# CederGroupHub/chgnet

Measured on NVIDIA H100. Metric: structures_per_sec_EFS, higher is better.
Workload: dtype f32

## Files before the change

chgnet_b200/_lib.py:

```python
from __future__ import annotations

import ctypes
import os
from ctypes import c_char_p, c_float, c_int32, c_int64, c_void_p

import torch
from torch import Tensor

_HERE = os.path.dirname(os.path.abspath(__file__))
LIB_PATH = os.path.join(_HERE, "libchgnet_b200.so")

P, I, F, I64 = c_void_p, c_int32, c_float, c_int64

SIGNATURES: dict[str, list] = {
    "chg_embed_atoms": [P, P, I, P, P],
    "chg_edge_geometry": [P, P, P, P, P, P, I, P, P, P, P],
    "chg_bond_basis_embed": [P, P, I, P, P, I, F, F, I, P, P, P, P, P, P],
    "chg_bond_basis_bwd": [P, P, I, P, P, I, F, F, I, P, P, P, P, P, P, P],
    "chg_angle_basis_embed": [P, P, P, I, P, I, P, P, P, P],
    "chg_angle_basis_bwd": [P, P, P, I, P, I, P, P, P, P, P],
    "chg_linear": [P, P, I, I, P, P, P, P, I, P, P],
    "chg_gather_rows": [P, P, I, I, P, P],
    "chg_scatter_rows": [P, P, I, I, P, P],
    "chg_atom_conv_fwd": [P, P, P, P, P, P, I, P, P, P, P, P, P, P],
    "chg_atom_conv_bwd": [P, P, P, P, P, P, I, P, P, P, P, P, P, P, P, P],
    "chg_segment_sum": [P, I, P, P, I, I, I, P, I, P],
    "chg_atom_conv_fused": [P, P, P, P, P, P, P, I, I, P, P, P, P, P, P, P],
    "chg_bond_conv_fused": [P, P, P, P, P, P, P, P, I, I, P, P, P, P, P, P, P, P],
    "chg_bond_conv_fwd": [P, P, P, P, P, P, P, I, P, P, P, P, P, P, P],
    "chg_bond_conv_bwd": [P, P, P, P, P, I, P, P, P, P, P, P, P, P, P],
    "chg_angle_update_fwd": [P, P, P, P, P, P, P, I, P, P, P, P],
    "chg_angle_update_bwd": [P, P, I, P, P, P, P],
    "chg_readout": [P, P, P, I, P, P, P, P, I, P, F, P, P, P, P, P, P, P],
    "chg_magmom": [P, I, P, F, P, P],
    "chg_force_virial": [P, P, P, P, P, P, P, P, P, P, I, P, P, P],
    "chg_wgrad": [P, P, I, P, I, P, I, P, I, I, P, I, P, P, P],
    "chg_colsum": [P, I, P, I, P, I, I, P, P],
    "chg_readout_bwd": [P, I, P, P, P, P, I, P, P, P, P, P, P, P, P],
    "chg_magmom_bwd": [P, I, P, F, P, P, P, P],
    "chg_loss_terms": [P, P, I, I, F, P, P, P],
    "chg_adam_step": [P, P, P, P, I64, F, F, F, F, F, I, P],
    "chg_edge_tangent": [P, P, P, P, P, P, P, P, I, P, P, P],
    "chg_bond_basis_tangent": [P, P, P, I, P, P, I, F, F, I, P, P, P, P, P, P],
    "chg_bond_basis_bwd2": [P, P, P, I, P, P, I, F, F, I, P, P, P, P, P, P],
    "chg_angle_basis_tangent": [P, P, P, P, I, P, I, P, P, P, P],
    "chg_angle_basis_bwd2": [P, P, P, P, I, P, I, P, P, P, P],
    "chg_atom_conv_tan": [P, P, P, P, P, P, P, I, P, P, P, P, P, P, P, P],
# ... 169 lines not shown

    def segment_sum(self, data, perm, ptr, accumulate, out):
        self._chk(data, perm, ptr)
        if not out.is_cuda or out.stride(1) != 1:
            raise ChgnetB200Error("segment_sum output must be a CUDA tensor with unit column stride")
        n_items = data.shape[0] if perm is None else perm.shape[0]
        self._call("chg_segment_sum", _p(data), data.shape[1], _p(perm), _p(ptr), ptr.shape[0] - 1, n_items,
                   int(accumulate), _p(out), out.stride(0))

    def bond_conv_fwd(self, pij, px, pa, wbg, ang_atom, ang_i, ang_j, w2t, b2, ln, upd, save_pre, save_p):
        self._chk(pij, px, pa, wbg, ang_atom, ang_i, ang_j, w2t, b2, ln, upd, save_pre, save_p)
        self._call("chg_bond_conv_fwd", _p(pij), _p(px), _p(pa), _p(wbg), _p(ang_atom), _p(ang_i), _p(ang_j),
                   ang_i.shape[0], _p(w2t), _p(b2), _p(ln), _p(upd), _p(save_pre), _p(save_p))

    def bond_conv_bwd(self, save_pre, save_p, wbg, ang_i, ang_j, g_agg, w2, ln, g_pre, gw_i, gw_j, g_p=None,
                      g_ln=None):
        self._chk(save_pre, save_p, wbg, ang_i, ang_j, g_agg, w2, ln, g_pre, gw_i, gw_j, g_p, g_ln)
        self._call("chg_bond_conv_bwd", _p(save_pre), _p(save_p), _p(wbg), _p(ang_i), _p(ang_j), ang_i.shape[0],
                   _p(g_agg), _p(w2), _p(ln), _p(g_pre), _p(gw_i), _p(gw_j), _p(g_p), _p(g_ln))

    def angle_update_fwd(self, pij, px, pa, ang, ang_atom, ang_i, ang_j, ln, ang_new, save_p):
        self._chk(pij, px, pa, ang, ang_atom, ang_i, ang_j, ln, ang_new, save_p)
        self._call("chg_angle_update_fwd", _p(pij), _p(px), _p(pa), _p(ang), _p(ang_atom), _p(ang_i), _p(ang_j),
                   ang_i.shape[0], _p(ln), _p(ang_new), _p(save_p))

    def angle_update_bwd(self, save_p, g_ang_in, ln, g_pre, g_ln=None):
        self._chk(save_p, g_ang_in, ln, g_pre, g_ln)
        self._call("chg_angle_update_bwd", _p(save_p), _p(g_ang_in), save_p.shape[0], _p(ln), _p(g_pre), _p(g_ln))

    @staticmethod
    def _chk_rows(*tensors: Tensor | None) -> None:
        for t in tensors:
            if t is not None and (not t.is_cuda or t.stride(-1) != 1):
                raise ChgnetB200Error("kernel arguments must be CUDA tensors with unit column stride")

    def _workspace(self, n_out: int, device) -> Tensor:
        ws = getattr(self, "_ws", None)
        if ws is None or ws.device != device:
            need = max(int(self.lib.chg_wgrad_workspace_floats(n)) for n in (64, 128, 256))
            ws = torch.empty(need, dtype=torch.float32, device=device)
            self._ws = ws
# ... 151 lines not shown
```

chgnet_b200/csrc/gated.cu:

```cuda
#include <cstdlib>

#include "gated_common.cuh"

namespace chg {
namespace {

using namespace gated;

template <int MODE>
struct FwdSmem {
  static constexpr bool HAS_W2 = MODE != ANGLE;
  static constexpr int W2_OFF = 0;
  static constexpr int TILE_OFF = W2_OFF + (HAS_W2 ? 64 * 128 : 0);
  static constexpr int TILE_FLOATS = HAS_W2 ? TM * HS : 0;
  static constexpr int B2_OFF = TILE_OFF + TILE_FLOATS;
  static constexpr int LN_OFF = B2_OFF + 128;
  static constexpr int IDX_OFF = LN_OFF + 256;
  static constexpr int TOTAL_BYTES = (IDX_OFF + 3 * TM) * 4;
};

template <int MODE>
__global__ void __launch_bounds__(NTHR, 2) gated_fwd_kernel(const FwdArgs a) {
  using L = FwdSmem<MODE>;
  extern __shared__ __align__(16) float smem[];
// ... 125 lines not shown
  const int tid = threadIdx.x;
  const int tx = tid & 15, ty = tid >> 4;
  const int r0 = ty * 4, c0 = tx * 4;
  const bool use_ln = a.ln != nullptr;

  if (L::HAS_W2) copy_to_smem(s_w2, a.w2, 128 * 64, tid);
  if (use_ln) s_ln[tid] = a.ln[tid];
  float ln_acc[16];
#pragma unroll
  for (int j = 0; j < 16; ++j) ln_acc[j] = 0.f;

  const int n_tiles = (a.n_rows + TM - 1) / TM;
  for (int tile = blockIdx.x; tile < n_tiles; tile += gridDim.x) {
    const int base = tile * TM;
    __syncthreads();
    if (MODE != ANGLE && tid < TM) {
      const int r = min(base + tid, a.n_rows - 1);
      s_idx[tid] = a.idx0[r];
      s_idx[TM + tid] = a.idx1[r];
      if (MODE == ATOM) s_idx[2 * TM + tid] = a.idx2[r];
    }
    __syncthreads();

    float4 g1, g2, b1, b2v;
    if (use_ln) {
      g1 = lds4(s_ln + c0);
      b1 = lds4(s_ln + 64 + c0);
      g2 = lds4(s_ln + 128 + c0);
      b2v = lds4(s_ln + 192 + c0);
    }
#pragma unroll
    for (int i = 0; i < 4; ++i) {
      const int row = r0 + i;
      const int g = base + row;
      const bool valid = g < a.n_rows;
      const int r = min(g, a.n_rows - 1);
      const float4 pc4 = ldg4(a.save_p + (size_t)r * 128 + c0);
      const float4 pg4 = ldg4(a.save_p + (size_t)r * 128 + 64 + c0);
      float y1[4] = {pc4.x, pc4.y, pc4.z, pc4.w};
      float y2[4] = {pg4.x, pg4.y, pg4.z, pg4.w};
      float xh1[4], xh2[4], rstd1 = 1.f, rstd2 = 1.f;
      if (use_ln) {
        ln_stats(y1, xh1, rstd1);
        ln_stats(y2, xh2, rstd2);
#pragma unroll
        for (int j = 0; j < 4; ++j) {
          y1[j] = fmaf(xh1[j], f4at(g1, j), f4at(b1, j));
          y2[j] = fmaf(xh2[j], f4at(g2, j), f4at(b2v, j));
        }
      }
      float s1[4], core[4], gate[4];
      float4 o;
#pragma unroll
// ... 579 lines not shown
  CHG_CHECK_ARG(pij && px && pa && ang && ang_atom && ang_i && ang_j && ang_new, "null pointer");
  FwdArgs a{pij, px, pa, ang, nullptr, ang_i, ang_j, ang_atom, n_angles, nullptr, nullptr, ln, ang_new,
            nullptr, save_p};
  return launch_fwd<ANGLE>(a, as_stream(stream));
}

extern "C" int chg_angle_update_bwd(const float* save_p, const float* g_ang_in, int32_t n_angles, const float* ln,
                                    float* g_pre, double* g_ln, void* stream) {
  CHG_CHECK_ARG(n_angles >= 0, "negative size");
  if (n_angles == 0) return CHG_OK;
  CHG_CHECK_ARG(save_p && g_pre, "null pointer");
  BwdArgs a{nullptr, nullptr, nullptr, nullptr, nullptr, nullptr, n_angles, nullptr, save_p, g_ang_in,
            nullptr, ln, g_pre, nullptr, nullptr, nullptr, g_ln};
  return launch_bwd<ANGLE>(a, as_stream(stream));
}
```

chgnet_b200/csrc/gated_common.cuh:

```cuda
#pragma once
#include "common.cuh"

namespace chg {
namespace gated {

constexpr int HS = 132;
constexpr float LN_EPS = 1e-5f;
}
int ws_min_rows();
namespace gated {

enum Mode { ATOM = 0, BOND = 1, ANGLE = 2 };

struct FwdArgs {
  const float* p_a;
  const float* p_b;
  const float* p_c;
  const float* feat;
  const float* wgt;
  const int32_t* idx0;
  const int32_t* idx1;
  const int32_t* idx2;
  int32_t n_rows;
  const float* w2t;
// ... 10 lines not shown
  const float* wgt;
  const int32_t* idx0;
  const int32_t* idx1;
  const int32_t* idx2;
  int32_t n_rows;
  const float* save_pre;
  const float* save_p;
  const float* g_in;
  const float* w2;
  const float* ln;
  float* g_pre;
  float* g_w0;
  float* g_w1;
  float* g_p;
  double* g_ln;
};

__device__ __forceinline__ void ln_stats(const float (&v)[4], float (&xhat)[4], float& rstd) {
  const float mean = sum16(v[0] + v[1] + v[2] + v[3]) * (1.f / 64.f);
  float d[4], ss = 0.f;
#pragma unroll
  for (int j = 0; j < 4; ++j) {
    d[j] = v[j] - mean;
    ss = fmaf(d[j], d[j], ss);
  }
  const float var = sum16(ss) * (1.f / 64.f);
  rstd = 1.f / sqrtf(var + LN_EPS);
#pragma unroll
  for (int j = 0; j < 4; ++j) xhat[j] = d[j] * rstd;
}
// ... 94 lines not shown
```

chgnet_b200/csrc/gated_ws.cu:

```cuda
#include "gated_common.cuh"
#include "tc.cuh"

namespace chg {
namespace gated {
namespace {

constexpr int WS_THREADS = 512;
constexpr int TR = 128;
constexpr int HALF_BYTES = TR * 64 * 4;
constexpr int IMG_BYTES = 64 * 64 * 4;
constexpr int STRIP = 16;

struct WsSmem {
  static constexpr int IMG_OFF = 0;
  static constexpr int HS_OFF = 4 * IMG_BYTES;
  static constexpr int O_OFF = HS_OFF + 2 * HALF_BYTES;
  static constexpr int GIDX_OFF = O_OFF + HALF_BYTES;
  static constexpr int EIDX_OFF = GIDX_OFF + 2 * 3 * TR * 4;
  static constexpr int B2_OFF = EIDX_OFF + 4 * TR * 4;
  static constexpr int LN_OFF = B2_OFF + 128 * 4;
  static constexpr int TOTAL = LN_OFF + 256 * 4;
};

struct WsBars {
// ... 353 lines not shown
struct WsBwdSmem {
  static constexpr int IMG_OFF = 0;
  static constexpr int T1_OFF = 4 * IMG_BYTES;
  static constexpr int T2_OFF = T1_OFF + 2 * HALF_BYTES;
  static constexpr int PIDX_OFF = T2_OFF + 2 * HALF_BYTES;
  static constexpr int FIDX_OFF = PIDX_OFF + 3 * TR * 4;
  static constexpr int LN_OFF = FIDX_OFF + 3 * TR * 4;
  static constexpr int TOTAL = LN_OFF + 256 * 4;
};

struct WsBwdBars {
  uint64_t a_full, a_empty;
};

template <int MODE>
__global__ void __launch_bounds__(WS_THREADS, 1) gated_ws_bwd_kernel(const BwdArgs a) {
  extern __shared__ __align__(1024) uint8_t smem_raw[];
  uint8_t* s_img = smem_raw + WsBwdSmem::IMG_OFF;
  uint8_t* s_t1 = smem_raw + WsBwdSmem::T1_OFF;
  uint8_t* s_t2 = smem_raw + WsBwdSmem::T2_OFF;
  int* s_pidx = reinterpret_cast<int*>(smem_raw + WsBwdSmem::PIDX_OFF);
  int* s_fidx = reinterpret_cast<int*>(smem_raw + WsBwdSmem::FIDX_OFF);
  float* s_ln = reinterpret_cast<float*>(smem_raw + WsBwdSmem::LN_OFF);
  __shared__ __align__(8) WsBwdBars bars;

  const int tid = threadIdx.x, warp = tid >> 5;
  const bool use_ln = a.ln != nullptr;
  const int n_tiles = (a.n_rows + TR - 1) / TR;

  build_image_ws(s_img, s_img + IMG_BYTES, a.w2, 64, 0, tid);
// ... 34 lines not shown
      if (use_ln) {
        g1 = lds4(s_ln + c0);
        b1 = lds4(s_ln + 64 + c0);
        g2 = lds4(s_ln + 128 + c0);
        b2v = lds4(s_ln + 192 + c0);
      }
      tc::mbar_wait(&bars.a_empty, (tl & 1) ^ 1);
#pragma unroll 2
      for (int pass = 0; pass < 8; ++pass) {
        const int row = pass * 16 + ty;
        const int g = base + row;
        const bool valid = g < a.n_rows;
        const int r = min(g, a.n_rows - 1);
        const float4 pc4 = ldg4(a.save_p + (size_t)r * 128 + c0);
        const float4 pg4 = ldg4(a.save_p + (size_t)r * 128 + 64 + c0);
        float4 gm, wv;
        if (MODE == ATOM) {
          gm = ldg4(a.g_in + (size_t)s_pidx[row] * 64 + c0);
          wv = ldg4(a.wgt + (size_t)s_pidx[2 * TR + row] * 64 + c0);
        } else {
          gm = ldg4(a.g_in + (size_t)s_pidx[row] * 64 + c0);
          wv = ldg4(a.wgt + (size_t)s_pidx[row] * 64 + c0);
        }
        float y1[4] = {pc4.x, pc4.y, pc4.z, pc4.w};
        float y2[4] = {pg4.x, pg4.y, pg4.z, pg4.w};
        float xh1[4], xh2[4], rstd1 = 1.f, rstd2 = 1.f;
        if (use_ln) {
          ln_stats(y1, xh1, rstd1);
          ln_stats(y2, xh2, rstd2);
#pragma unroll
          for (int j = 0; j < 4; ++j) {
            y1[j] = fmaf(xh1[j], f4at(g1, j), f4at(b1, j));
            y2[j] = fmaf(xh2[j], f4at(g2, j), f4at(b2v, j));
          }
        }
        float s1[4], core[4], gate[4];
        float4 o;
#pragma unroll
        for (int j = 0; j < 4; ++j) {
          s1[j] = sigmoid_f(y1[j]);
          core[j] = y1[j] * s1[j];
          gate[j] = sigmoid_f(y2[j]);
          f4at(o, j) = core[j] * gate[j];
        }
        float4 go;
        if (MODE == ATOM) {
          if (valid) stg4(a.g_w0 + (size_t)g * 64 + c0, gm * o);
          go = gm * wv;
        } else {
          const float4 wj = ldg4(a.wgt + (size_t)s_pidx[TR + row] * 64 + c0);
          const float4 gmo = gm * o;
          if (valid) {
            stg4(a.g_w0 + (size_t)g * 64 + c0, gmo * wj);
            stg4(a.g_w1 + (size_t)g * 64 + c0, gmo * wv);
          }
          go = gm * wv * wj;
        }
        float gy1[4], gy2[4];
#pragma unroll
        for (int j = 0; j < 4; ++j) {
          const float gj = f4at(go, j);
          gy1[j] = gj * gate[j] * (s1[j] * fmaf(y1[j], 1.f - s1[j], 1.f));
          gy2[j] = gj * core[j] * gate[j] * (1.f - gate[j]);
        }
        if (use_ln) {
          float gx[4], sa = 0.f, sb = 0.f;
#pragma unroll
          for (int j = 0; j < 4; ++j) {
            gx[j] = gy1[j] * f4at(g1, j);
            sa += gx[j];
            sb = fmaf(gx[j], xh1[j], sb);
          }
          sa = sum16(sa) * (1.f / 64.f);
          sb = sum16(sb) * (1.f / 64.f);
#pragma unroll
          for (int j = 0; j < 4; ++j) gy1[j] = rstd1 * (gx[j] - sa - xh1[j] * sb);
          sa = 0.f, sb = 0.f;
#pragma unroll
          for (int j = 0; j < 4; ++j) {
            gx[j] = gy2[j] * f4at(g2, j);
            sa += gx[j];
            sb = fmaf(gx[j], xh2[j], sb);
          }
          sa = sum16(sa) * (1.f / 64.f);
          sb = sum16(sb) * (1.f / 64.f);
#pragma unroll
          for (int j = 0; j < 4; ++j) gy2[j] = rstd2 * (gx[j] - sa - xh2[j] * sb);
        }
        *reinterpret_cast<float4*>(s_t1 + swz(row, tx)) = make_float4(gy1[0], gy1[1], gy1[2], gy1[3]);
        *reinterpret_cast<float4*>(s_t1 + HALF_BYTES + swz(row, tx)) = make_float4(gy2[0], gy2[1], gy2[2], gy2[3]);
      }
      tc::wg_barrier(1, 256);
      tc::mbar_arrive(&bars.a_full);
    }
  } else {
    const int t = tid - 256;
    const int tx = t & 15, ty = t >> 4;
    const int c0 = tx * 4;
    const int crow = t & 127, chalf = t >> 7;
    const int row0 = ((warp - 8) >> 2) * 64;
    const uint32_t img = tc::smem_u32(s_img);
    int tl = 0;
    for (int tile = blockIdx.x; tile < n_tiles; tile += gridDim.x, ++tl) {
// ... 59 lines not shown
}

template <int MODE>
int launch_ws_bwd(const BwdArgs& a, cudaStream_t stream) {
  if (a.n_rows == 0) return CHG_OK;
  static bool attr_set = false;
  if (!attr_set) {
    CHG_CUDA(cudaFuncSetAttribute(gated_ws_bwd_kernel<MODE>, cudaFuncAttributeMaxDynamicSharedMemorySize, WsBwdSmem::TOTAL));
    attr_set = true;
  }
  const int n_tiles = (a.n_rows + TR - 1) / TR;
  gated_ws_bwd_kernel<MODE><<<min(n_tiles, sm_count()), WS_THREADS, WsBwdSmem::TOTAL, stream>>>(a);
  CHG_LAUNCH_END();
}

}

int atom_conv_bwd_ws(const BwdArgs& a, cudaStream_t stream) { return launch_ws_bwd<ATOM>(a, stream); }
int bond_conv_bwd_ws(const BwdArgs& a, cudaStream_t stream) { return launch_ws_bwd<BOND>(a, stream); }

}
}
```

chgnet_b200/csrc/native_engine.cu:

```cuda
#include <cstdarg>
#include <cstdio>
#include <cstring>
#include <string>

#include "common.cuh"

namespace chg {
namespace {

constexpr size_t ALIGN = 256;
constexpr int64_t PAD = 16;

struct GatedW {
  const float *w2t = nullptr, *w2 = nullptr, *b2 = nullptr, *ln = nullptr;
  const float *a_t = nullptr, *b_t = nullptr, *c_t = nullptr, *bias1 = nullptr;
  const float *a_b = nullptr, *b_b = nullptr, *c_b = nullptr;
  const float *wo_t = nullptr, *wo = nullptr, *bo = nullptr;
};
struct Weights {
  const float *emb, *freq_ag, *freq_bg, *freq_ang, *w3t, *w3, *wang_t, *wang;
  GatedW atom[CHG_MAX_CONV], bond[CHG_MAX_CONV], angle[CHG_MAX_CONV];
  const float *readout_ln, *mlp_wt, *mlp_w, *mlp_b, *w_last, *w_mag, *atom_ref;
};

// ... 170 lines not shown
  float *rvec = c.f(true, (size_t)Ed * 3), *dist = c.f(true, Ed), *rhat = c.f(true, (size_t)Ed * 3);
  RUN(c, "edge_geometry", chg_edge_geometry(b.frac, b.lattice, b.owner, b.center, b.nbr, b.image, Ed, rvec, dist, rhat, st));
  float *e = c.f(true, (size_t)Eu * 64), *wag = c.f(true, (size_t)Eu * 64), *wbg = c.f(true, (size_t)Eu * 64);
  RUN(c, "bond_basis_embed", chg_bond_basis_embed(dist, b.u2d, Eu, W.freq_ag, W.freq_bg, hp.num_radial, hp.atom_graph_cutoff,
                                                  hp.bond_graph_cutoff, hp.cutoff_coeff, W.w3t, e, wag, wbg, nullptr, st));
  float *ang = nullptr, *ang_alt = nullptr, *wbg_s = nullptr;
  if (has_ang) {
    ang = c.f(true, (size_t)A * 64);
    ang_alt = c.f(true, (size_t)A * 64);
    RUN(c, "angle_basis_embed", chg_angle_basis_embed(rhat, b.ang_di, b.ang_dj, A, W.freq_ang, (hp.num_angular - 1) / 2,
                                                      W.wang_t, ang, nullptr, st));
    wbg_s = c.f(true, (size_t)Es * 64);
    RUN(c, "gather_rows", chg_gather_rows(wbg, b.short_ids, Es, 64, wbg_s, st));
  }
  struct SavedAtom { float *pcn, *pe, *p; } sa[CHG_MAX_CONV];
  struct SavedBond { float *pre, *p; } sb[CHG_MAX_CONV];
  float* sang[CHG_MAX_CONV];

  auto atom_conv = [&](int t, const float* xin, float* xout) {
    const GatedW& g = W.atom[t];
    float* pcn = c.f(grad, (size_t)N * 256);
    float* pe = c.f(grad, (size_t)Eu * 128);
    lin(xin, nullptr, N, 64, g.a_t, nullptr, nullptr, nullptr, 256, pcn);
    lin(e, nullptr, Eu, 64, g.b_t, g.bias1, nullptr, nullptr, 128, pe);
    float* save_p = grad ? c.f(true, (size_t)Ed * 128) : nullptr;
    float* agg = c.f(false, (size_t)N * 64);
    float* work = c.f(false, (size_t)chg_gated_fused_workspace_floats(Ed));
    RUN(c, "atom_conv_fused", chg_atom_conv_fused(pcn, pe, wag, b.center, b.nbr, b.d2u, b.ptr_c, Ed, N, g.w2t, g.b2, g.ln, agg, save_p,
                                                  work, st));
    sa[t] = SavedAtom{pcn, pe, save_p};
    lin(agg, nullptr, N, 64, g.wo_t, g.bo, xin, nullptr, 64, xout);
    c.ar.reset_tmp();
  };

  float* x_mag = nullptr;
  for (int t = 0; t < n_conv - 1; ++t) {
    float* xn = (t == n_conv - 2 && o.atom_fea != nullptr) ? o.atom_fea : c.f(true, (size_t)N * 64);
    atom_conv(t, x, xn);
    x = xn;
    if (has_ang) {
      const GatedW& g = W.bond[t];
      float* pij = c.f(false, (size_t)Es * 256);
      float* px = c.f(false, (size_t)N * 128);
      float* pa = c.f(false, (size_t)A * 128);
      lin(e, b.short_ids, Es, 64, g.a_t, g.bias1, nullptr, nullptr, 256, pij);
      lin(x, nullptr, N, 64, g.b_t, nullptr, nullptr, nullptr, 128, px);
      lin(ang, nullptr, A, 64, g.c_t, nullptr, nullptr, nullptr, 128, pa);
      float* s_pre = grad ? c.f(true, (size_t)A * 128) : nullptr;
      float* s_p = grad ? c.f(true, (size_t)A * 128) : nullptr;
      float* agg = c.f(false, (size_t)Es * 64);
      float* work = c.f(false, (size_t)chg_gated_fused_workspace_floats(A));
      RUN(c, "bond_conv_fused", chg_bond_conv_fused(pij, px, pa, wbg_s, b.ang_atom, b.ang_is, b.ang_js, b.ptr_is, A, Es, g.w2t, g.b2,
                                                    g.ln, agg, s_pre, s_p, work, st));
      lin(agg, nullptr, Es, 64, g.wo_t, g.bo, e, b.short_ids, 64, e);
      sb[t] = SavedBond{s_pre, s_p};
      c.ar.reset_tmp();
      if (t < n_conv - 2) {
        const GatedW& ga = W.angle[t];
        pij = c.f(false, (size_t)Es * 256);
        px = c.f(false, (size_t)N * 128);
        pa = c.f(false, (size_t)A * 128);
        lin(e, b.short_ids, Es, 64, ga.a_t, ga.bias1, nullptr, nullptr, 256, pij);
        lin(x, nullptr, N, 64, ga.b_t, nullptr, nullptr, nullptr, 128, px);
        lin(ang, nullptr, A, 64, ga.c_t, nullptr, nullptr, nullptr, 128, pa);
        float* s_pa = grad ? c.f(true, (size_t)A * 128) : nullptr;
        RUN(c, "angle_update_fwd", chg_angle_update_fwd(pij, px, pa, ang, b.ang_atom, b.ang_is, b.ang_js, A, ga.ln, ang_alt, s_pa, st));
        sang[t] = s_pa;
        float* sw = ang;
        ang = ang_alt;
        ang_alt = sw;
        c.ar.reset_tmp();
      }
    }
    if (t == n_conv - 2) {
      x_mag = x;
      if (o.magmom != nullptr) RUN(c, "magmom", chg_magmom(x, N, W.w_mag, hp.b_mag, o.magmom, st));
    }
  }
  if (n_conv == 1 && o.magmom != nullptr) c.zero(o.magmom, (size_t)N * 4);
  (void)x_mag;
  {
    float* xn = c.f(true, (size_t)N * 64);
// ... 43 lines not shown
    float* sp = c.f(false, (size_t)Es * 256);
    seg(g_pre, 128, nullptr, b.ptr_is, Es, A, 0, sp, 256);
    seg(g_pre, 128, b.perm_js, b.ptr_js, Es, A, 0, sp + 128, 256);
    lin(sp, nullptr, Es, 256, g.a_b, nullptr, g_e, b.short_ids, 64, g_e);
    float* spx = c.f(false, (size_t)N * 128);
    seg(g_pre, 128, b.perm_x, b.ptr_x, N, A, 0, spx, 128);
    lin(spx, nullptr, N, 128, g.b_b, nullptr, g_x, nullptr, 64, g_x);
  };

  atom_bwd(n_conv - 1);
  for (int t = n_conv - 2; t >= 0; --t) {
    if (has_ang) {
      if (t < n_conv - 2) {
        const GatedW& ga = W.angle[t];
        float* g_pre = c.f(false, (size_t)A * 128);
        RUN(c, "angle_update_bwd", chg_angle_update_bwd(sang[t], g_a_live ? g_a : nullptr, A, ga.ln, g_pre, nullptr, st));
        lin(g_pre, nullptr, A, 128, ga.c_b, nullptr, g_a_live ? g_a : nullptr, nullptr, 64, g_a);
        g_a_live = true;
        angle_scatter(g_pre, ga);
        c.ar.reset_tmp();
      }
      const GatedW& g = W.bond[t];
      float* g_agg = c.f(false, (size_t)Es * 64);
      lin(g_e, b.short_ids, Es, 64, g.wo, nullptr, nullptr, nullptr, 64, g_agg);
      float* g_pre = c.f(false, (size_t)A * 128);
      float *gw_i = c.f(false, (size_t)A * 64), *gw_j = c.f(false, (size_t)A * 64);
      RUN(c, "bond_conv_bwd", chg_bond_conv_bwd(sb[t].pre, sb[t].p, wbg_s, b.ang_is, b.ang_js, A, g_agg, g.w2, g.ln, g_pre, gw_i,
                                                gw_j, nullptr, nullptr, st));
      lin(g_pre, nullptr, A, 128, g.c_b, nullptr, g_a_live ? g_a : nullptr, nullptr, 64, g_a);
      g_a_live = true;
      angle_scatter(g_pre, g);
      seg(gw_i, 64, nullptr, b.ptr_is, Es, A, 1, g_wbg, 64);
      seg(gw_j, 64, b.perm_js, b.ptr_js, Es, A, 1, g_wbg, 64);
      c.ar.reset_tmp();
    }
    atom_bwd(t);
  }

  float* g_dist = c.f(false, Eu);
  float* g_wbg_full = c.f(false, (size_t)Eu * 64);
  c.zero(g_wbg_full, (size_t)Eu * 256);
  if (has_ang) RUN(c, "scatter_rows", chg_scatter_rows(g_wbg, b.short_ids, Es, 64, g_wbg_full, st));
  RUN(c, "bond_basis_bwd", chg_bond_basis_bwd(dist, b.u2d, Eu, W.freq_ag, W.freq_bg, hp.num_radial, hp.atom_graph_cutoff,
// ... 155 lines not shown
```

include/chgnet_b200.h:

```cpp
#ifndef CHGNET_B200_H
#define CHGNET_B200_H

#include <stdint.h>

#ifdef __cplusplus
extern "C" {
#endif

#define CHG_FEA 64
#define CHG_MAX_CONV 8
#define CHG_MAX_Z 94
#define CHG_OK 0
#define CHG_ERR_ARG (-1)
#define CHG_ERR_CUDA (-2)

const char* chg_last_error(void);
int chg_abi_version(void);
int64_t chg_launch_count(void);
int chg_set_option(const char* name, int32_t value);

int chg_embed_atoms(const int32_t* z, const float* emb, int32_t n_atoms, float* x, void* stream);

int chg_edge_geometry(const float* frac, const float* lattice, const int32_t* atom_owner,
                      const int32_t* center, const int32_t* nbr, const float* image,
// ... 56 lines not shown
int chg_bond_conv_fused(const float* pij, const float* px, const float* pa, const float* wbg,
                        const int32_t* ang_atom, const int32_t* ang_i, const int32_t* ang_j,
                        const int32_t* ptr_i, int32_t n_angles, int32_t n_slots, const float* w2t,
                        const float* b2, const float* ln, float* agg, float* save_pre, float* save_p,
                        float* work, void* stream);

int chg_bond_conv_fwd(const float* pij, const float* px, const float* pa, const float* wbg,
                      const int32_t* ang_atom, const int32_t* ang_i, const int32_t* ang_j,
                      int32_t n_angles, const float* w2t, const float* b2, const float* ln,
                      float* upd, float* save_pre, float* save_p, void* stream);
int chg_bond_conv_bwd(const float* save_pre, const float* save_p, const float* wbg,
                      const int32_t* ang_i, const int32_t* ang_j, int32_t n_angles,
                      const float* g_agg, const float* w2, const float* ln, float* g_pre,
                      float* gw_i, float* gw_j, float* g_p ,
                      double* g_ln , void* stream);

int chg_angle_update_fwd(const float* pij, const float* px, const float* pa, const float* ang,
                         const int32_t* ang_atom, const int32_t* ang_i, const int32_t* ang_j,
                         int32_t n_angles, const float* ln, float* ang_new, float* save_p,
                         void* stream);
int chg_angle_update_bwd(const float* save_p, const float* g_ang_in, int32_t n_angles,
                         const float* ln, float* g_pre, double* g_ln ,
                         void* stream);

int chg_readout(const float* x, const int32_t* z, const int32_t* atom_owner, int32_t n_atoms,
                const float* ln, const float* mlp_wt, const float* mlp_w, const float* mlp_b,
                int32_t n_hidden, const float* w_last, float b_last, const float* atom_ref,
                float* site_e, float* h_out, double* e_graph, double* e_ref, float* g_x,
                void* stream);
int chg_magmom(const float* x, int32_t n_atoms, const float* w, float b, float* m, void* stream);

int chg_force_virial(const float* rvec, const float* dist, const float* rhat,
                     const double* g_rhat, const float* g_dist, const int32_t* d2u,
                     const int32_t* u2d, const int32_t* center, const int32_t* nbr,
                     const int32_t* atom_owner, int32_t n_edges, double* force,
                     double* virial, void* stream);

typedef struct {
// ... 202 lines not shown
```

Before: 9931.

## Rematerialise gated pre-activations in bond/angle backward instead of saving them

Instead of writing per-angle pre-activation and gated-product buffers (A×128 floats each) during the forward pass, the forward now keeps the smaller factor products (pij, px, pa) and the backward kernels re-gather and recompute the pre-activations. A new bond backward kernel recomputes the w2 GEMM on tensor cores within the tile before applying the gate derivative. The angle-update backward gains a remat path that gathers products directly. This trades extra gathers and a GEMM recompute for reduced global memory writes and reads of large per-angle saved activations.

```diff
diff --git a/chgnet_b200/_lib.py b/chgnet_b200/_lib.py
--- a/chgnet_b200/_lib.py
+++ b/chgnet_b200/_lib.py
@@ -31,6 +31,8 @@
     "chg_bond_conv_bwd": [P, P, P, P, P, I, P, P, P, P, P, P, P, P, P],
     "chg_angle_update_fwd": [P, P, P, P, P, P, P, I, P, P, P, P],
     "chg_angle_update_bwd": [P, P, I, P, P, P, P],
+    "chg_bond_conv_bwd_remat": [P, P, P, P, P, P, P, I, P, P, P, P, P, P, P, P, P],
+    "chg_angle_update_bwd_remat": [P, P, P, P, P, P, P, I, P, P, P, P],
     "chg_readout": [P, P, P, I, P, P, P, P, I, P, F, P, P, P, P, P, P, P],
     "chg_magmom": [P, I, P, F, P, P],
     "chg_force_virial": [P, P, P, P, P, P, P, P, P, P, I, P, P, P],
@@ -230,7 +232,14 @@
                    ang_i.shape[0], _p(w2t), _p(b2), _p(ln), _p(upd), _p(save_pre), _p(save_p))
 
     def bond_conv_bwd(self, save_pre, save_p, wbg, ang_i, ang_j, g_agg, w2, ln, g_pre, gw_i, gw_j, g_p=None,
-                      g_ln=None):
+                      g_ln=None, pij=None, px=None, pa=None, ang_atom=None, w2t=None, b2=None):
+        if pij is not None:
+            if g_p is not None or g_ln is not None:
+                raise ChgnetB200Error("bond_conv_bwd: the rematerialising reverse has no training outputs")
+            self._chk(pij, px, pa, wbg, ang_atom, ang_i, ang_j, g_agg, w2t, b2, w2, ln, g_pre, gw_i, gw_j)
+            self._call("chg_bond_conv_bwd_remat", _p(pij), _p(px), _p(pa), _p(wbg), _p(ang_atom), _p(ang_i), _p(ang_j),
+                       ang_i.shape[0], _p(g_agg), _p(w2t), _p(b2), _p(w2), _p(ln), _p(g_pre), _p(gw_i), _p(gw_j))
+            return
         self._chk(save_pre, save_p, wbg, ang_i, ang_j, g_agg, w2, ln, g_pre, gw_i, gw_j, g_p, g_ln)
         self._call("chg_bond_conv_bwd", _p(save_pre), _p(save_p), _p(wbg), _p(ang_i), _p(ang_j), ang_i.shape[0],
                    _p(g_agg), _p(w2), _p(ln), _p(g_pre), _p(gw_i), _p(gw_j), _p(g_p), _p(g_ln))
@@ -240,7 +249,13 @@
         self._call("chg_angle_update_fwd", _p(pij), _p(px), _p(pa), _p(ang), _p(ang_atom), _p(ang_i), _p(ang_j),
                    ang_i.shape[0], _p(ln), _p(ang_new), _p(save_p))
 
-    def angle_update_bwd(self, save_p, g_ang_in, ln, g_pre, g_ln=None):
+    def angle_update_bwd(self, save_p, g_ang_in, ln, g_pre, g_ln=None, pij=None, px=None, pa=None, ang_atom=None,
+                         ang_i=None, ang_j=None):
+        if pij is not None:
+            self._chk(pij, px, pa, ang_atom, ang_i, ang_j, g_ang_in, ln, g_pre, g_ln)
+            self._call("chg_angle_update_bwd_remat", _p(pij), _p(px), _p(pa), _p(ang_atom), _p(ang_i), _p(ang_j),
+                       _p(g_ang_in), g_pre.shape[0], _p(ln), _p(g_pre), _p(g_ln))
+            return
         self._chk(save_p, g_ang_in, ln, g_pre, g_ln)
         self._call("chg_angle_update_bwd", _p(save_p), _p(g_ang_in), save_p.shape[0], _p(ln), _p(g_pre), _p(g_ln))
 
diff --git a/chgnet_b200/csrc/gated.cu b/chgnet_b200/csrc/gated.cu
--- a/chgnet_b200/csrc/gated.cu
+++ b/chgnet_b200/csrc/gated.cu
@@ -163,11 +163,12 @@
   for (int tile = blockIdx.x; tile < n_tiles; tile += gridDim.x) {
     const int base = tile * TM;
     __syncthreads();
-    if (MODE != ANGLE && tid < TM) {
+    const bool remat = MODE == ANGLE && a.save_p == nullptr;
+    if ((MODE != ANGLE || remat) && tid < TM) {
       const int r = min(base + tid, a.n_rows - 1);
       s_idx[tid] = a.idx0[r];
       s_idx[TM + tid] = a.idx1[r];
-      if (MODE == ATOM) s_idx[2 * TM + tid] = a.idx2[r];
+      if (MODE != BOND) s_idx[2 * TM + tid] = a.idx2[r];
     }
     __syncthreads();
 
@@ -178,14 +179,22 @@
       g2 = lds4(s_ln + 128 + c0);
       b2v = lds4(s_ln + 192 + c0);
     }
+    float p_re[4][8];
+    if (remat) {
+#pragma unroll
+      for (int i = 0; i < 4; ++i)
+#pragma unroll
+        for (int j = 0; j < 8; ++j) p_re[i][j] = 0.f;
+      gather_pre<TM>(p_re, a.p_a, a.p_b, a.p_c, s_idx, base, a.n_rows, r0, c0);
+    }
 #pragma unroll
     for (int i = 0; i < 4; ++i) {
       const int row = r0 + i;
       const int g = base + row;
       const bool valid = g < a.n_rows;
       const int r = min(g, a.n_rows - 1);
-      const float4 pc4 = ldg4(a.save_p + (size_t)r * 128 + c0);
-      const float4 pg4 = ldg4(a.save_p + (size_t)r * 128 + 64 + c0);
+      const float4 pc4 = remat ? make_float4(p_re[i][0], p_re[i][1], p_re[i][2], p_re[i][3]) : ldg4(a.save_p + (size_t)r * 128 + c0);
+      const float4 pg4 = remat ? make_float4(p_re[i][4], p_re[i][5], p_re[i][6], p_re[i][7]) : ldg4(a.save_p + (size_t)r * 128 + 64 + c0);
       float y1[4] = {pc4.x, pc4.y, pc4.z, pc4.w};
       float y2[4] = {pg4.x, pg4.y, pg4.z, pg4.w};
       float xh1[4], xh2[4], rstd1 = 1.f, rstd2 = 1.f;
@@ -795,3 +804,14 @@
             nullptr, ln, g_pre, nullptr, nullptr, nullptr, g_ln};
   return launch_bwd<ANGLE>(a, as_stream(stream));
 }
+
+extern "C" int chg_angle_update_bwd_remat(const float* pij, const float* px, const float* pa, const int32_t* ang_atom,
+                                          const int32_t* ang_i, const int32_t* ang_j, const float* g_ang_in, int32_t n_angles,
+                                          const float* ln, float* g_pre, double* g_ln, void* stream) {
+  CHG_CHECK_ARG(n_angles >= 0, "negative size");
+  if (n_angles == 0) return CHG_OK;
+  CHG_CHECK_ARG(pij && px && pa && ang_atom && ang_i && ang_j && g_pre, "null pointer");
+  BwdArgs a{pij, px, nullptr, ang_i, ang_j, ang_atom, n_angles, nullptr, nullptr, g_ang_in,
+            nullptr, ln, g_pre, nullptr, nullptr, nullptr, g_ln, pa};
+  return launch_bwd<ANGLE>(a, as_stream(stream));
+}
diff --git a/chgnet_b200/csrc/gated_common.cuh b/chgnet_b200/csrc/gated_common.cuh
--- a/chgnet_b200/csrc/gated_common.cuh
+++ b/chgnet_b200/csrc/gated_common.cuh
@@ -48,6 +48,7 @@
   float* g_w1;
   float* g_p;
   double* g_ln;
+  const float* p_c;
 };
 
 __device__ __forceinline__ void ln_stats(const float (&v)[4], float (&xhat)[4], float& rstd) {
diff --git a/chgnet_b200/csrc/gated_ws.cu b/chgnet_b200/csrc/gated_ws.cu
--- a/chgnet_b200/csrc/gated_ws.cu
+++ b/chgnet_b200/csrc/gated_ws.cu
@@ -391,6 +391,75 @@
 };
 
 template <int MODE>
+__device__ __forceinline__ void gate_bwd_row(const float4 pc4, const float4 pg4, const float4 gm, const float4 wv, const float4 wj,
+                                             bool use_ln, const float4 g1, const float4 b1, const float4 g2, const float4 b2v,
+                                             float* gw0, float* gw1, float (&gy1)[4], float (&gy2)[4]) {
+  float y1[4] = {pc4.x, pc4.y, pc4.z, pc4.w};
+  float y2[4] = {pg4.x, pg4.y, pg4.z, pg4.w};
+  float xh1[4], xh2[4], rstd1 = 1.f, rstd2 = 1.f;
+  if (use_ln) {
+    ln_stats(y1, xh1, rstd1);
+    ln_stats(y2, xh2, rstd2);
+#pragma unroll
+    for (int j = 0; j < 4; ++j) {
+      y1[j] = fmaf(xh1[j], f4at(g1, j), f4at(b1, j));
+      y2[j] = fmaf(xh2[j], f4at(g2, j), f4at(b2v, j));
+    }
+  }
+  float s1[4], core[4], gate[4];
+  float4 o;
+#pragma unroll
+  for (int j = 0; j < 4; ++j) {
+    s1[j] = sigmoid_f(y1[j]);
+    core[j] = y1[j] * s1[j];
+    gate[j] = sigmoid_f(y2[j]);
+    f4at(o, j) = core[j] * gate[j];
+  }
+  float4 go;
+  if (MODE == ATOM) {
+    if (gw0 != nullptr) stg4(gw0, gm * o);
+    go = gm * wv;
+  } else {
+    const float4 gmo = gm * o;
+    if (gw0 != nullptr) {
+      stg4(gw0, gmo * wj);
+      stg4(gw1, gmo * wv);
+    }
+    go = gm * wv * wj;
+  }
+#pragma unroll
+  for (int j = 0; j < 4; ++j) {
+    const float gj = f4at(go, j);
+    gy1[j] = gj * gate[j] * (s1[j] * fmaf(y1[j], 1.f - s1[j], 1.f));
+    gy2[j] = gj * core[j] * gate[j] * (1.f - gate[j]);
+  }
+  if (use_ln) {
+    float gx[4], sa = 0.f, sb = 0.f;
+#pragma unroll
+    for (int j = 0; j < 4; ++j) {
+      gx[j] = gy1[j] * f4at(g1, j);
+      sa += gx[j];
+      sb = fmaf(gx[j], xh1[j], sb);
+    }
+    sa = sum16(sa) * (1.f / 64.f);
+    sb = sum16(sb) * (1.f / 64.f);
+#pragma unroll
+    for (int j = 0; j < 4; ++j) gy1[j] = rstd1 * (gx[j] - sa - xh1[j] * sb);
+    sa = 0.f, sb = 0.f;
+#pragma unroll
+    for (int j = 0; j < 4; ++j) {
+      gx[j] = gy2[j] * f4at(g2, j);
+      sa += gx[j];
+      sb = fmaf(gx[j], xh2[j], sb);
+    }
+    sa = sum16(sa) * (1.f / 64.f);
+    sb = sum16(sb) * (1.f / 64.f);
+#pragma unroll
+    for (int j = 0; j < 4; ++j) gy2[j] = rstd2 * (gx[j] - sa - xh2[j] * sb);
+  }
+}
+
+template <int MODE>
 __global__ void __launch_bounds__(WS_THREADS, 1) gated_ws_bwd_kernel(const BwdArgs a) {
   extern __shared__ __align__(1024) uint8_t smem_raw[];
   uint8_t* s_img = smem_raw + WsBwdSmem::IMG_OFF;
@@ -455,79 +524,12 @@
         const int r = min(g, a.n_rows - 1);
         const float4 pc4 = ldg4(a.save_p + (size_t)r * 128 + c0);
         const float4 pg4 = ldg4(a.save_p + (size_t)r * 128 + 64 + c0);
-        float4 gm, wv;
-        if (MODE == ATOM) {
-          gm = ldg4(a.g_in + (size_t)s_pidx[row] * 64 + c0);
-          wv = ldg4(a.wgt + (size_t)s_pidx[2 * TR + row] * 64 + c0);
-        } else {
-          gm = ldg4(a.g_in + (size_t)s_pidx[row] * 64 + c0);
-          wv = ldg4(a.wgt + (size_t)s_pidx[row] * 64 + c0);
-        }
-        float y1[4] = {pc4.x, pc4.y, pc4.z, pc4.w};
-        float y2[4] = {pg4.x, pg4.y, pg4.z, pg4.w};
-        float xh1[4], xh2[4], rstd1 = 1.f, rstd2 = 1.f;
-        if (use_ln) {
-          ln_stats(y1, xh1, rstd1);
-          ln_stats(y2, xh2, rstd2);
-#pragma unroll
-          for (int j = 0; j < 4; ++j) {
-            y1[j] = fmaf(xh1[j], f4at(g1, j), f4at(b1, j));
-            y2[j] = fmaf(xh2[j], f4at(g2, j), f4at(b2v, j));
-          }
-        }
-        float s1[4], core[4], gate[4];
-        float4 o;
-#pragma unroll
-        for (int j = 0; j < 4; ++j) {
-          s1[j] = sigmoid_f(y1[j]);
-          core[j] = y1[j] * s1[j];
-          gate[j] = sigmoid_f(y2[j]);
-          f4at(o, j) = core[j] * gate[j];
-        }
-        float4 go;
-        if (MODE == ATOM) {
-          if (valid) stg4(a.g_w0 + (size_t)g * 64 + c0, gm * o);
-          go = gm * wv;
-        } else {
-          const float4 wj = ldg4(a.wgt + (size_t)s_pidx[TR + row] * 64 + c0);
-          const float4 gmo = gm * o;
-          if (valid) {
-            stg4(a.g_w0 + (size_t)g * 64 + c0, gmo * wj);
-            stg4(a.g_w1 + (size_t)g * 64 + c0, gmo * wv);
-          }
-          go = gm * wv * wj;
-        }
+        const float4 gm = ldg4(a.g_in + (size_t)s_pidx[row] * 64 + c0);
+        const float4 wv = ldg4(a.wgt + (size_t)s_pidx[MODE == ATOM ? 2 * TR + row : row] * 64 + c0);
+        const float4 wj = MODE == ATOM ? wv : ldg4(a.wgt + (size_t)s_pidx[TR + row] * 64 + c0);
         float gy1[4], gy2[4];
-#pragma unroll
-        for (int j = 0; j < 4; ++j) {
-          const float gj = f4at(go, j);
-          gy1[j] = gj * gate[j] * (s1[j] * fmaf(y1[j], 1.f - s1[j], 1.f));
-          gy2[j] = gj * core[j] * gate[j] * (1.f - gate[j]);
-        }
-        if (use_ln) {
-          float gx[4], sa = 0.f, sb = 0.f;
-#pragma unroll
-          for (int j = 0; j < 4; ++j) {
-            gx[j] = gy1[j] * f4at(g1, j);
-            sa += gx[j];
-            sb = fmaf(gx[j], xh1[j], sb);
-          }
-          sa = sum16(sa) * (1.f / 64.f);
-          sb = sum16(sb) * (1.f / 64.f);
-#pragma unroll
-          for (int j = 0; j < 4; ++j) gy1[j] = rstd1 * (gx[j] - sa - xh1[j] * sb);
-          sa = 0.f, sb = 0.f;
-#pragma unroll
-          for (int j = 0; j < 4; ++j) {
-            gx[j] = gy2[j] * f4at(g2, j);
-            sa += gx[j];
-            sb = fmaf(gx[j], xh2[j], sb);
-          }
-          sa = sum16(sa) * (1.f / 64.f);
-          sb = sum16(sb) * (1.f / 64.f);
-#pragma unroll
-          for (int j = 0; j < 4; ++j) gy2[j] = rstd2 * (gx[j] - sa - xh2[j] * sb);
-        }
+        gate_bwd_row<MODE>(pc4, pg4, gm, wv, wj, use_ln, g1, b1, g2, b2v, valid ? a.g_w0 + (size_t)g * 64 + c0 : nullptr,
+                           MODE == BOND && valid ? a.g_w1 + (size_t)g * 64 + c0 : nullptr, gy1, gy2);
         *reinterpret_cast<float4*>(s_t1 + swz(row, tx)) = make_float4(gy1[0], gy1[1], gy1[2], gy1[3]);
         *reinterpret_cast<float4*>(s_t1 + HALF_BYTES + swz(row, tx)) = make_float4(gy2[0], gy2[1], gy2[2], gy2[3]);
       }
@@ -617,6 +619,170 @@
   CHG_LAUNCH_END();
 }
 
+constexpr int RR = 64;
+constexpr int R_HALF_BYTES = RR * 64 * 4;
+
+struct RematArgs {
+  const float *pij, *px, *pa, *wbg;
+  const int32_t *ang_atom, *ang_i, *ang_j;
+  int32_t n_rows;
+  const float *g_agg, *w2t, *b2, *w2, *ln;
+  float *g_pre, *gw_i, *gw_j;
+};
+
+struct RematSmem {
+  static constexpr int IMG_OFF = 0;
+  static constexpr int T_OFF = 8 * IMG_BYTES;
+  static constexpr int IDX_OFF = T_OFF + 2 * 2 * R_HALF_BYTES;
+  static constexpr int B2_OFF = IDX_OFF + 2 * 3 * RR * 4;
+  static constexpr int LN_OFF = B2_OFF + 128 * 4;
+  static constexpr int TOTAL = LN_OFF + 256 * 4;
+};
+
+__global__ void __launch_bounds__(WS_THREADS, 1) bond_bwd_remat_kernel(const RematArgs a) {
+  extern __shared__ __align__(1024) uint8_t smem_raw[];
+  uint8_t* s_img = smem_raw + RematSmem::IMG_OFF;
+  float* s_b2 = reinterpret_cast<float*>(smem_raw + RematSmem::B2_OFF);
+  float* s_ln = reinterpret_cast<float*>(smem_raw + RematSmem::LN_OFF);
+
+  const int tid = threadIdx.x, warp = tid >> 5;
+  const int part = warp >> 3, pt = tid & 255;
+  const int tx = pt & 15, ty = pt >> 4;
+  const int c0 = tx * 4;
+  const bool use_ln = a.ln != nullptr;
+  const int n_tiles = (a.n_rows + RR - 1) / RR;
+  uint8_t* s_t = smem_raw + RematSmem::T_OFF + part * 2 * R_HALF_BYTES;
+  int* s_idx = reinterpret_cast<int*>(smem_raw + RematSmem::IDX_OFF) + part * 3 * RR;
+
+  build_image_ws(s_img, s_img + IMG_BYTES, a.w2t, 128, 0, tid);
+  build_image_ws(s_img + 2 * IMG_BYTES, s_img + 3 * IMG_BYTES, a.w2t, 128, 64, tid);
+  build_image_ws(s_img + 4 * IMG_BYTES, s_img + 5 * IMG_BYTES, a.w2, 64, 0, tid);
+  build_image_ws(s_img + 6 * IMG_BYTES, s_img + 7 * IMG_BYTES, a.w2 + 64 * 64, 64, 0, tid);
+  if (tid < 128) s_b2[tid] = a.b2[tid];
+  if (tid < 256) s_ln[tid] = use_ln ? a.ln[tid] : 0.f;
+  tc::fence_async_smem();
+  __syncthreads();
+
+  float4 g1, b1, g2, b2v;
+  if (use_ln) {
+    g1 = lds4(s_ln + c0);
+    b1 = lds4(s_ln + 64 + c0);
+    g2 = lds4(s_ln + 128 + c0);
+    b2v = lds4(s_ln + 192 + c0);
+  }
+  auto sync = [&]() { tc::wg_barrier(1 + part, 256); };
+  const int wh = (warp >> 2) & 1;
+  uint8_t* s_half = s_t + wh * R_HALF_BYTES;
+  const uint32_t img = tc::smem_u32(s_img);
+  auto tile_at = [&](int r, int k) { return *reinterpret_cast<const float*>(s_half + swz(r, k >> 2) + (k & 3) * 4); };
+  auto store_frag = [&](const float (&d)[32]) {
+    __syncwarp();
+#pragma unroll
+    for (int i = 0; i < 32; i += 2) {
+      const int r = tc::frag_row(i), c = tc::frag_col(i);
+      *reinterpret_cast<float2*>(s_half + swz(r, c >> 2) + (c & 3) * 4) = make_float2(d[i], d[i + 1]);
+    }
+  };
+
+  const int stride = 2 * gridDim.x;
+  for (int tile = 2 * blockIdx.x + part; tile < n_tiles; tile += stride) {
+    const int base = tile * RR;
+    if (pt < RR) {
+      const int r = min(base + pt, a.n_rows - 1);
+      const int si = a.ang_i[r], sj = a.ang_j[r];
+      s_idx[pt] = si;
+      s_idx[RR + pt] = sj;
+      s_idx[2 * RR + pt] = a.ang_atom[r];
+      prefetch_l2(a.g_agg + (size_t)si * 64);
+      prefetch_l2(a.g_agg + (size_t)si * 64 + 32);
+      prefetch_l2(a.wbg + (size_t)si * 64);
+      prefetch_l2(a.wbg + (size_t)si * 64 + 32);
+      prefetch_l2(a.wbg + (size_t)sj * 64);
+      prefetch_l2(a.wbg + (size_t)sj * 64 + 32);
+    } else if (pt < 3 * RR) {
+      const int nt = tile + stride;
+      if (nt < n_tiles) {
+        const int u = pt - RR;
+        const float* row = a.pa + (size_t)min(nt * RR + (u & 63), a.n_rows - 1) * 128 + (u >> 6) * 64;
+        prefetch_l2(row);
+        prefetch_l2(row + 32);
+      }
+    }
+    sync();
+
+    auto gather = [&](int row, int col) {
+      const float* s0 = a.pij + (size_t)s_idx[row] * 256 + col + c0;
+      const float* s1 = a.pij + (size_t)s_idx[RR + row] * 256 + 128 + col + c0;
+      const float* s2 = a.px + (size_t)s_idx[2 * RR + row] * 128 + col + c0;
+      const float* s3 = a.pa + (size_t)min(base + row, a.n_rows - 1) * 128 + col + c0;
+      return ldg4(s0) + ldg4(s1) + ldg4(s2) + ldg4(s3);
+    };
+#pragma unroll 2
+    for (int pass = 0; pass < 4; ++pass) {
+      const int row = pass * 16 + ty;
+      const float4 vc = gather(row, 0), vg = gather(row, 64);
+      *reinterpret_cast<float4*>(s_t + swz(row, tx)) = make_float4(silu_f(vc.x), silu_f(vc.y), silu_f(vc.z), silu_f(vc.w));
+      *reinterpret_cast<float4*>(s_t + R_HALF_BYTES + swz(row, tx)) =
+          make_float4(silu_f(vg.x), silu_f(vg.y), silu_f(vg.z), silu_f(vg.w));
+    }
+    sync();
+
+    {
+      float d[32];
+#pragma unroll
+      for (int i = 0; i < 32; ++i) d[i] = 0.f;
+      tc::wg_gemm_k64<64>(d, tile_at, img + (2 * wh) * IMG_BYTES, img + (2 * wh + 1) * IMG_BYTES, 2048);
+#pragma unroll
+      for (int i = 0; i < 32; ++i) d[i] += s_b2[wh * 64 + tc::frag_col(i)];
+      store_frag(d);
+    }
+    sync();
+
+#pragma unroll 2
+    for (int pass = 0; pass < 4; ++pass) {
+      const int row = pass * 16 + ty;
+      const int g = base + row;
+      const bool valid = g < a.n_rows;
+      const float4 pc4 = *reinterpret_cast<const float4*>(s_t + swz(row, tx));
+      const float4 pg4 = *reinterpret_cast<const float4*>(s_t + R_HALF_BYTES + swz(row, tx));
+      const float4 gm = ldg4(a.g_agg + (size_t)s_idx[row] * 64 + c0);
+      const float4 wv = ldg4(a.wbg + (size_t)s_idx[row] * 64 + c0);
+      const float4 wj = ldg4(a.wbg + (size_t)s_idx[RR + row] * 64 + c0);
+      float gy1[4], gy2[4];
+      gate_bwd_row<BOND>(pc4, pg4, gm, wv, wj, use_ln, g1, b1, g2, b2v, valid ? a.gw_i + (size_t)g * 64 + c0 : nullptr,
+                         valid ? a.gw_j + (size_t)g * 64 + c0 : nullptr, gy1, gy2);
+      *reinterpret_cast<float4*>(s_t + swz(row, tx)) = make_float4(gy1[0], gy1[1], gy1[2], gy1[3]);
+      *reinterpret_cast<float4*>(s_t + R_HALF_BYTES + swz(row, tx)) = make_float4(gy2[0], gy2[1], gy2[2], gy2[3]);
+    }
+    sync();
+
+    {
+      float d[32];
+#pragma unroll
+      for (int i = 0; i < 32; ++i) d[i] = 0.f;
+      tc::wg_gemm_k64<64>(d, tile_at, img + (4 + 2 * wh) * IMG_BYTES, img + (5 + 2 * wh) * IMG_BYTES, 2048);
+      store_frag(d);
+    }
+    sync();
+
+#pragma unroll 2
+    for (int pass = 0; pass < 4; ++pass) {
+      const int row = pass * 16 + ty;
+      const int g = base + row;
+      const float4 hc = *reinterpret_cast<const float4*>(s_t + swz(row, tx));
+      const float4 hg = *reinterpret_cast<const float4*>(s_t + R_HALF_BYTES + swz(row, tx));
+      const float4 vc = gather(row, 0), vg = gather(row, 64);
+      if (g < a.n_rows) {
+        stg4(a.g_pre + (size_t)g * 128 + c0,
+             make_float4(hc.x * dsilu_f(vc.x), hc.y * dsilu_f(vc.y), hc.z * dsilu_f(vc.z), hc.w * dsilu_f(vc.w)));
+        stg4(a.g_pre + (size_t)g * 128 + 64 + c0,
+             make_float4(hg.x * dsilu_f(vg.x), hg.y * dsilu_f(vg.y), hg.z * dsilu_f(vg.z), hg.w * dsilu_f(vg.w)));
+      }
+    }
+    sync();
+  }
+}
+
 }
 
 int atom_conv_bwd_ws(const BwdArgs& a, cudaStream_t stream) { return launch_ws_bwd<ATOM>(a, stream); }
@@ -624,3 +790,23 @@
 
 }
 }
+
+extern "C" int chg_bond_conv_bwd_remat(const float* pij, const float* px, const float* pa, const float* wbg,
+                                       const int32_t* ang_atom, const int32_t* ang_i, const int32_t* ang_j, int32_t n_angles,
+                                       const float* g_agg, const float* w2t, const float* b2, const float* w2, const float* ln,
+                                       float* g_pre, float* gw_i, float* gw_j, void* stream) {
+  using namespace chg::gated;
+  CHG_CHECK_ARG(n_angles >= 0, "negative size");
+  if (n_angles == 0) return CHG_OK;
+  CHG_CHECK_ARG(pij && px && pa && wbg && ang_atom && ang_i && ang_j && g_agg && w2t && b2 && w2 && g_pre && gw_i && gw_j,
+                "null pointer");
+  static bool attr_set = false;
+  if (!attr_set) {
+    CHG_CUDA(cudaFuncSetAttribute(bond_bwd_remat_kernel, cudaFuncAttributeMaxDynamicSharedMemorySize, RematSmem::TOTAL));
+    attr_set = true;
+  }
+  const RematArgs a{pij, px, pa, wbg, ang_atom, ang_i, ang_j, n_angles, g_agg, w2t, b2, w2, ln, g_pre, gw_i, gw_j};
+  const int n_pairs = (n_angles + 2 * RR - 1) / (2 * RR);
+  bond_bwd_remat_kernel<<<min(n_pairs, chg::sm_count()), WS_THREADS, RematSmem::TOTAL, chg::as_stream(stream)>>>(a);
+  CHG_LAUNCH_END();
+}
diff --git a/chgnet_b200/csrc/native_engine.cu b/chgnet_b200/csrc/native_engine.cu
--- a/chgnet_b200/csrc/native_engine.cu
+++ b/chgnet_b200/csrc/native_engine.cu
@@ -3,7 +3,7 @@
 #include <cstring>
 #include <string>
 
-#include "common.cuh"
+#include "gated_common.cuh"
 
 namespace chg {
 namespace {
@@ -208,8 +208,9 @@
     RUN(c, "gather_rows", chg_gather_rows(wbg, b.short_ids, Es, 64, wbg_s, st));
   }
   struct SavedAtom { float *pcn, *pe, *p; } sa[CHG_MAX_CONV];
-  struct SavedBond { float *pre, *p; } sb[CHG_MAX_CONV];
-  float* sang[CHG_MAX_CONV];
+  struct SavedProducts { float *pij, *px, *pa; } sang[CHG_MAX_CONV];
+  struct SavedBond { float *pij, *px, *pa, *pre, *p; } sb[CHG_MAX_CONV];
+  const bool bond_remat = gated_impl() == 3 && A >= ws_min_rows();
 
   auto atom_conv = [&](int t, const float* xin, float* xout) {
     const GatedW& g = W.atom[t];
@@ -234,32 +235,32 @@
     x = xn;
     if (has_ang) {
       const GatedW& g = W.bond[t];
-      float* pij = c.f(false, (size_t)Es * 256);
-      float* px = c.f(false, (size_t)N * 128);
-      float* pa = c.f(false, (size_t)A * 128);
+      const bool keep_products = grad && bond_remat;
+      float* pij = c.f(keep_products, (size_t)Es * 256);
+      float* px = c.f(keep_products, (size_t)N * 128);
+      float* pa = c.f(keep_products, (size_t)A * 128);
       lin(e, b.short_ids, Es, 64, g.a_t, g.bias1, nullptr, nullptr, 256, pij);
       lin(x, nullptr, N, 64, g.b_t, nullptr, nullptr, nullptr, 128, px);
       lin(ang, nullptr, A, 64, g.c_t, nullptr, nullptr, nullptr, 128, pa);
-      float* s_pre = grad ? c.f(true, (size_t)A * 128) : nullptr;
-      float* s_p = grad ? c.f(true, (size_t)A * 128) : nullptr;
+      float* s_pre = grad && !bond_remat ? c.f(true, (size_t)A * 128) : nullptr;
+      float* s_p = grad && !bond_remat ? c.f(true, (size_t)A * 128) : nullptr;
       float* agg = c.f(false, (size_t)Es * 64);
       float* work = c.f(false, (size_t)chg_gated_fused_workspace_floats(A));
       RUN(c, "bond_conv_fused", chg_bond_conv_fused(pij, px, pa, wbg_s, b.ang_atom, b.ang_is, b.ang_js, b.ptr_is, A, Es, g.w2t, g.b2,
                                                     g.ln, agg, s_pre, s_p, work, st));
       lin(agg, nullptr, Es, 64, g.wo_t, g.bo, e, b.short_ids, 64, e);
-      sb[t] = SavedBond{s_pre, s_p};
+      sb[t] = SavedBond{pij, px, pa, s_pre, s_p};
       c.ar.reset_tmp();
       if (t < n_conv - 2) {
         const GatedW& ga = W.angle[t];
-        pij = c.f(false, (size_t)Es * 256);
-        px = c.f(false, (size_t)N * 128);
-        pa = c.f(false, (size_t)A * 128);
+        pij = c.f(grad, (size_t)Es * 256);
+        px = c.f(grad, (size_t)N * 128);
+        pa = c.f(grad, (size_t)A * 128);
         lin(e, b.short_ids, Es, 64, ga.a_t, ga.bias1, nullptr, nullptr, 256, pij);
         lin(x, nullptr, N, 64, ga.b_t, nullptr, nullptr, nullptr, 128, px);
         lin(ang, nullptr, A, 64, ga.c_t, nullptr, nullptr, nullptr, 128, pa);
-        float* s_pa = grad ? c.f(true, (size_t)A * 128) : nullptr;
-        RUN(c, "angle_update_fwd", chg_angle_update_fwd(pij, px, pa, ang, b.ang_atom, b.ang_is, b.ang_js, A, ga.ln, ang_alt, s_pa, st));
-        sang[t] = s_pa;
+        RUN(c, "angle_update_fwd", chg_angle_update_fwd(pij, px, pa, ang, b.ang_atom, b.ang_is, b.ang_js, A, ga.ln, ang_alt, nullptr, st));
+        sang[t] = SavedProducts{pij, px, pa};
         float* sw = ang;
         ang = ang_alt;
         ang_alt = sw;
@@ -333,7 +334,8 @@
       if (t < n_conv - 2) {
         const GatedW& ga = W.angle[t];
         float* g_pre = c.f(false, (size_t)A * 128);
-        RUN(c, "angle_update_bwd", chg_angle_update_bwd(sang[t], g_a_live ? g_a : nullptr, A, ga.ln, g_pre, nullptr, st));
+        RUN(c, "angle_update_bwd", chg_angle_update_bwd_remat(sang[t].pij, sang[t].px, sang[t].pa, b.ang_atom, b.ang_is, b.ang_js,
+                                                              g_a_live ? g_a : nullptr, A, ga.ln, g_pre, nullptr, st));
         lin(g_pre, nullptr, A, 128, ga.c_b, nullptr, g_a_live ? g_a : nullptr, nullptr, 64, g_a);
         g_a_live = true;
         angle_scatter(g_pre, ga);
@@ -344,8 +346,12 @@
       lin(g_e, b.short_ids, Es, 64, g.wo, nullptr, nullptr, nullptr, 64, g_agg);
       float* g_pre = c.f(false, (size_t)A * 128);
       float *gw_i = c.f(false, (size_t)A * 64), *gw_j = c.f(false, (size_t)A * 64);
-      RUN(c, "bond_conv_bwd", chg_bond_conv_bwd(sb[t].pre, sb[t].p, wbg_s, b.ang_is, b.ang_js, A, g_agg, g.w2, g.ln, g_pre, gw_i,
-                                                gw_j, nullptr, nullptr, st));
+      if (bond_remat)
+        RUN(c, "bond_conv_bwd", chg_bond_conv_bwd_remat(sb[t].pij, sb[t].px, sb[t].pa, wbg_s, b.ang_atom, b.ang_is, b.ang_js, A, g_agg,
+                                                        g.w2t, g.b2, g.w2, g.ln, g_pre, gw_i, gw_j, st));
+      else
+        RUN(c, "bond_conv_bwd", chg_bond_conv_bwd(sb[t].pre, sb[t].p, wbg_s, b.ang_is, b.ang_js, A, g_agg, g.w2, g.ln, g_pre, gw_i,
+                                                  gw_j, nullptr, nullptr, st));
       lin(g_pre, nullptr, A, 128, g.c_b, nullptr, g_a_live ? g_a : nullptr, nullptr, 64, g_a);
       g_a_live = true;
       angle_scatter(g_pre, g);
diff --git a/include/chgnet_b200.h b/include/chgnet_b200.h
--- a/include/chgnet_b200.h
+++ b/include/chgnet_b200.h
@@ -94,6 +94,10 @@
                       const float* g_agg, const float* w2, const float* ln, float* g_pre,
                       float* gw_i, float* gw_j, float* g_p ,
                       double* g_ln , void* stream);
+int chg_bond_conv_bwd_remat(const float* pij, const float* px, const float* pa, const float* wbg,
+                            const int32_t* ang_atom, const int32_t* ang_i, const int32_t* ang_j, int32_t n_angles,
+                            const float* g_agg, const float* w2t, const float* b2, const float* w2, const float* ln,
+                            float* g_pre, float* gw_i, float* gw_j, void* stream);
 
 int chg_angle_update_fwd(const float* pij, const float* px, const float* pa, const float* ang,
                          const int32_t* ang_atom, const int32_t* ang_i, const int32_t* ang_j,
@@ -102,6 +106,9 @@
 int chg_angle_update_bwd(const float* save_p, const float* g_ang_in, int32_t n_angles,
                          const float* ln, float* g_pre, double* g_ln ,
                          void* stream);
+int chg_angle_update_bwd_remat(const float* pij, const float* px, const float* pa, const int32_t* ang_atom,
+                               const int32_t* ang_i, const int32_t* ang_j, const float* g_ang_in, int32_t n_angles,
+                               const float* ln, float* g_pre, double* g_ln , void* stream);
 
 int chg_readout(const float* x, const int32_t* z, const int32_t* atom_owner, int32_t n_atoms,
                 const float* ln, const float* mlp_wt, const float* mlp_w, const float* mlp_b,
```

After: 10060 (median of 6 runs). +1.3%, better.
